# cvlab-yonsei/HVPR

Hardware: AMD Instinct MI355X
Metric: KITTI frames/sec/GPU (fwd, ~20k pts); VFE+scatter achieved HBM GB/s vs peak (higher is better)
Workload: dtype f32; 1 GPU; hvpr_car.yaml batch=1 forward-only, a1..a8 (on-GPU voxelize, pillar VFE, memory read-out + scatter, BEV backbone, head + decode, score top-k + rotated-BEV NMS); frames sharded over ranks, replicas only; global_batch=1, weights=deterministic synthetic (seed 0), BN stats randomised, cls bias -4.595

## Files before the change

### hvpr_amd/_lib.py

```python
import ctypes
import os

_HERE = os.path.dirname(os.path.abspath(__file__))
ABI_VERSION = 7
LIB_PATH = os.environ.get("HVPR_AMD_LIB", os.path.join(_HERE, "libhvpr_amd.so"))

_c = ctypes
_P = _c.c_void_p
_I = _c.c_int
_F = _c.c_float
_Z = _c.c_size_t
ALLREDUCE_FN = _c.CFUNCTYPE(_I, _P, _I, _P, _P)

SIGNATURES = {
    "hvpr_abi_version": (_I, []),
    "hvpr_status_string": (_c.c_char_p, [_I]),
    "hvpr_set_batchnorm_allreduce": (None, [_P, _P]),
    "hvpr_voxelize_workspace_bytes": (_Z, [_I, _I, _I, _I, _I]),
    "hvpr_voxelize_workspace_reset": (_I, [_P, _Z, _I, _I, _I, _I, _I, _P]),
    "hvpr_voxelize_workspace_status": (_I, [_P, _Z, _I, _I, _I, _I, _I, _P]),
    "hvpr_voxelize_f32": (_I, [_P, _I, _I, _I, _I, _P, _I, _F, _F, _F, _F, _F, _F, _I, _I, _I, _I, _I, _I,
                               _P, _P, _P, _P, _I, _P, _Z, _I, _I, _P]),
    "hvpr_pillar_vfe_fwd_f32": (_I, [_P, _P, _P, _I, _I, _P, _F, _F, _F, _F, _F, _F, _P, _P, _P, _P, _P, _P, _P, _P,
                                     _P, _P, _P, _P]),
# ... 37 lines not shown
    "hvpr_bn_relu_bwd_apply_nhwc_f32": (_I, [_P, _I, _I, _P, _c.c_longlong, _I, _P, _P, _P, _P, _I, _P, _P, _P, _P, _P, _c.c_double, _P]),
    "hvpr_memory_train_workspace_bytes": (_Z, [_I]),
    "hvpr_memory_train_fwd_f32": (_I, [_P, _c.c_longlong, _P, _I, _F, _P, _P, _P, _Z, _P]),
    "hvpr_memory_train_bwd_f32": (_I, [_P, _P, _c.c_longlong, _P, _I, _F, _P, _P, _P, _P, _P, _Z, _P]),
    "hvpr_point_pillar_topk_f32": (_I, [_P, _I, _P, _P, _I, _I, _P, _P]),
    "hvpr_scatter_add_rows_f32": (_I, [_P, _P, _c.c_longlong, _I, _I, _P, _P]),
    "hvpr_segment_sum_rows_f32": (_I, [_P, _c.c_longlong, _I, _I, _P, _P, _P, _c.c_longlong, _P, _c.c_longlong, _P]),
    "hvpr_fused_adam_truewd_f32": (_I, [_P, _P, _P, _P, _c.c_longlong, _F, _F, _F, _F, _F, _I, _P, _P]),
    "hvpr_assign_targets_workspace_bytes": (_Z, [_I, _I]),
    "hvpr_assign_targets_f32": (_I, [_P, _I, _P, _I, _I, _I, _I, _F, _F, _I, _I, _I, _c.c_longlong, _P, _P, _P, _P, _P, _Z, _P]),
    "hvpr_rpn_losses_workspace_bytes": (_Z, [_I, _c.c_longlong]),
    "hvpr_rpn_losses_f32": (_I, [_P, _P, _P, _P, _P, _P, _P, _I, _c.c_longlong, _I, _I, _F, _F, _F, _P, _F, _F, _F, _F, _P, _P, _P, _P,
                                 _P, _Z, _P]),
    "hvpr_mse_loss_workspace_bytes": (_Z, []),
    "hvpr_mse_loss_f32": (_I, [_P, _P, _c.c_longlong, _I, _F, _P, _P, _P, _Z, _P]),
    "hvpr_split_bf16_f32": (_I, [_P, _c.c_longlong, _I, _P, _P]),
    "hvpr_unsplit_bf16_f32": (_I, [_P, _c.c_longlong, _I, _P, _P]),
    "hvpr_conv2d_nhwc_bf16x3": (_I, [_P, _I, _I, _I, _I, _P, _P, _I, _I, _I, _I, _P, _P, _I, _P, _I, _I, _I, _I, _I, _P]),
    "hvpr_deconv_nhwc_bf16x3": (_I, [_P, _I, _I, _I, _I, _P, _P, _I, _I, _I, _I, _P, _I, _I, _I, _P]),
    "hvpr_point_flags_f32": (_I, [_P, _I, _I, _I, _P, _F, _P, _P, _I, _I, _P, _P]),
    "hvpr_compact_workspace_bytes": (_Z, [_I]),
    "hvpr_compact_rows_f32": (_I, [_P, _I, _I, _P, _P, _I, _P, _P, _Z, _P]),
    "hvpr_frame_offsets_f32": (_I, [_P, _I, _I, _I, _P, _P]),
    "hvpr_gather_rows_f32": (_I, [_P, _I, _I, _P, _I, _P, _P]),
    "hvpr_pillar_vfe_train_workspace_bytes": (_Z, []),
    "hvpr_pillar_vfe_train_fwd_f32": (_I, [_P, _P, _P, _I, _I, _P, _P, _P, _P, _P, _P, _F, _F, _F, _F, _F, _F, _F, _P, _P, _P, _P, _P, _P, _Z, _P]),
    "hvpr_pillar_vfe_bwd_f32": (_I, [_P, _P, _P, _I, _I, _P, _P, _P, _P, _P, _P, _F, _F, _F, _F, _F, _F, _F, _P, _P, _P, _P, _P, _P, _P, _P, _Z, _P]),
    "hvpr_conv2d_wino_wgrad_workspace_bytes": (_Z, [_I, _I, _I, _I, _I]),
    "hvpr_conv2d_wino_wgrad_nhwc_f32": (_I, [_P, _I, _I, _I, _I, _P, _I, _P, _P, _Z, _P]),
    "hvpr_conv2d_wino_packed_floats": (_Z, [_I, _I]),
    "hvpr_conv2d_wino_pack_f32": (_I, [_P, _P, _I, _I, _I, _P, _P]),
    "hvpr_conv2d_wino_nhwc_f32": (_I, [_P, _I, _I, _I, _I, _P, _P, _I, _I, _P, _P, _I, _P, _I, _I, _I, _P, _P]),
    "hvpr_conv2d_wino_stats_rows": (_I, [_I, _I, _I]),
    "hvpr_conv2d_s2_dgrad_nhwc_f32": (_I, [_P, _I, _I, _I, _I, _P, _P, _I, _I, _I, _I, _P, _I, _I, _P]),
    "hvpr_bn_train_affine_f32": (_I, [_P, _P, _P, _I, _P, _P, _F, _F, _P, _P, _P, _P, _P, _P]),
    "hvpr_bn_finalize_partials_f32": (_I, [_P, _I, _I, _c.c_longlong, _F, _P, _P, _P, _P]),
    "hvpr_conv2d_nhwc_f32": (_I, [_P, _I, _I, _I, _I, _P, _P, _I, _I, _I, _I, _I, _I, _P, _P, _I, _P, _I, _I, _I, _P]),
}

_lib = None


class HvprLibraryError(RuntimeError):
    pass


def lib():
    global _lib
    if _lib is None:
        if not os.path.exists(LIB_PATH):
            raise HvprLibraryError(
                f"{LIB_PATH} is missing: build it with `python -m hvpr_amd.build` (hipcc --offload-arch=gfx950). "
                "hvpr_amd has no CPU fallback.")
        try:
            L = ctypes.CDLL(LIB_PATH)
        except OSError as e:
            raise HvprLibraryError(f"cannot load {LIB_PATH}: {e}") from e
        for name, (res, args) in SIGNATURES.items():
            fn = getattr(L, name)
            fn.restype = res
            fn.argtypes = args
        if L.hvpr_abi_version() != ABI_VERSION:
            raise HvprLibraryError(f"{LIB_PATH} has ABI version {L.hvpr_abi_version()}, these wrappers need {ABI_VERSION}: "
                                   "rebuild it with `python -m hvpr_amd.build`")
        _lib = L
    return _lib
# ... 7 lines not shown
```

### hvpr_amd/bev_backbone.py

```python
import contextlib
import os

import torch
import torch.nn as nn

from . import kernels
from .folding import FoldCache, bn_scale_shift


class ConvLayer(nn.Module):

    def __init__(self, in_channels, out_channels, kernel_size, stride=1, padding=0, use_norm=True, activation=False):
        super().__init__()
        self.conv = nn.Conv2d(in_channels, out_channels, kernel_size=kernel_size, stride=stride, padding=padding)
        self.norm = nn.BatchNorm2d(out_channels, eps=1e-3, momentum=0.01) if use_norm else None
        self.relu = nn.ReLU() if activation else None


class SpatialAttention(nn.Module):

    def __init__(self):
        super().__init__()
        self.spatial = ConvLayer(2, 1, 3, stride=1, padding=1, use_norm=True, activation=False)

# ... 100 lines not shown
            cfg = _tile_cfg("trunk", i)
            lv = {"convs": []}
            sc, sh = bn_scale_shift(blk[2])
            wg = _wino_groups(i)
            lv["convs"].append(kernels.pack_conv_auto(blk[1].weight, sc, sh, stride=s, tile_cfg=cfg, px_groups=wg))
            for k in range(self.layer_nums[i]):
                sc, sh = bn_scale_shift(blk[5 + 3 * k])
                lv["convs"].append(kernels.pack_conv_auto(blk[4 + 3 * k].weight, sc, sh, tile_cfg=cfg, px_groups=wg))
            sc, sh = bn_scale_shift(self.sfmblocks_down[i][1])
            lv["sfm"] = kernels.pack_conv_auto(self.sfmblocks_down[i][0].weight, sc, sh, tile_cfg=_tile_cfg("sfm", i), px_groups=wg)
            planes = self.PRECISIONS[self.conv_precision]
            if planes:
                c3 = 4
                lv["convs3"] = []
                sc, sh = bn_scale_shift(blk[2])
                lv["convs3"].append(kernels.pack_conv_bf3(blk[1].weight, sc, sh, stride=s, tile_cfg=c3, planes=planes))
                for k in range(self.layer_nums[i]):
                    sc, sh = bn_scale_shift(blk[5 + 3 * k])
                    lv["convs3"].append(kernels.pack_conv_bf3(blk[4 + 3 * k].weight, sc, sh, tile_cfg=c3, planes=planes))
                sc, sh = bn_scale_shift(self.sfmblocks_down[i][1])
                lv["sfm3"] = kernels.pack_conv_bf3(self.sfmblocks_down[i][0].weight, sc, sh, tile_cfg=c3, planes=planes)
                de = self.deblocks[i]
                sc, sh = bn_scale_shift(de[1])
                lv["deconv3"] = kernels.pack_deconv_bf3(de[0].weight, sc, sh, planes=planes) \
                    if (planes == 2 and de[0].weight.shape[0] % 64 == 0) else None
            sl = self.scale_layers[i]
            sc, sh = bn_scale_shift(sl[2])
            lv["scale"] = kernels.pack_conv_auto(sl[1].weight, sc, sh, stride=s, tile_cfg=_tile_cfg("scale", i), px_groups=wg)
            de = self.deblocks[i]
            sc, sh = bn_scale_shift(de[1])
            us = int(self.upsample_strides[i])
            dcfg = _tile_cfg("deconv", i)
            lv["deconv"] = kernels.pack_deconv(de[0].weight, sc, sh, tile_cfg=dcfg)
            packed["levels"].append(lv)
        return packed

    def _forward_train(self, data_dict):
        if not data_dict["spatial_features"].is_cuda:
            raise RuntimeError("hvpr_amd: BaseBEVBackbone_Scale's training forward needs GPU tensors (the HIP path has no CPU fallback)")
        from . import conv_train as ct

        def nhwc(t):
            return t.permute(0, 2, 3, 1).contiguous()

        def cbr(seq, t, gate=None, resid=None):
            mods, k = list(seq), 0
            while k < len(mods):
                if isinstance(mods[k], nn.ZeroPad2d):
                    k += 1
                conv, bn = mods[k], mods[k + 1]
                last = k + 3 >= len(mods)
                if last and gate is not None and resid is t and conv.stride[0] == 1 and conv.kernel_size[0] == 3:
                    t = ct.sfm_step(t, conv.weight, bn, gate)
                else:
                    z, partials = ct.conv(t, conv.weight, conv.stride[0], stats=True)
                    t = ct.bn_relu(z, bn, gate=gate if last else None, resid=resid if last else None, partials=partials)
                k += 3
            return t

        def gate(y, uses):
            sp = self.attention.spatial
            g, mean, var = ct.spatial_gate_train(y, sp.conv.weight, sp.conv.bias, sp.norm.weight, sp.norm.bias, sp.norm.eps)
            ct.update_running_repeated(sp.norm, mean, var, ct.global_count(y.numel() // y.shape[-1], y.device), uses)
            return g

        x, xp = nhwc(data_dict["spatial_features"]), nhwc(data_dict["spatial_features_point"])
# ... 149 lines not shown
```

### hvpr_amd/csrc/conv_wino.hip

```cpp
#include <type_traits>

#include "common.h"

namespace {

typedef float f32x16 __attribute__((ext_vector_type(16)));
constexpr int KC = 8;
constexpr int BN = 64;
constexpr int TW = 16, PW = TW + 2;
constexpr int ROWP = 20;
constexpr int W_V4 = 16 * 2 * BN;

__device__ __forceinline__ void lds_dma16(const void *sbase_uniform, unsigned voff_bytes, unsigned lds_dst_uniform) {
    unsigned keep;
    asm volatile("s_mov_b32 %0, m0\n\ts_mov_b32 m0, %3\n\ts_nop 0\n\tglobal_load_lds_dwordx4 %1, %2\n\ts_mov_b32 m0, %0"
                 : "=&s"(keep)
                 : "v"(voff_bytes), "s"(sbase_uniform), "s"(lds_dst_uniform)
                 : "memory");
}

__device__ __forceinline__ unsigned lds_addr_of(const void *p) {
    return (unsigned)(size_t)(const __attribute__((address_space(3))) void *)p;
}

struct WinoArgs {
    const float *in;
    const float *wpk;
    const float *bias;
    float *out;
    const float *gate;
    const float *resid;
    int N, H, W, Cin;
    int cout, cout_pad;
    int out_cstride, out_coff, resid_cstride;
    int relu;
    int tiles_x, tiles_y, n_ct;
    float *stats;
};

__device__ __forceinline__ float4 f4_fma(float s, float4 a, float4 b) {
    return make_float4(fmaf(s, a.x, b.x), fmaf(s, a.y, b.y), fmaf(s, a.z, b.z), fmaf(s, a.w, b.w));
}
__device__ __forceinline__ float4 f4_add(float4 a, float4 b) { return make_float4(a.x + b.x, a.y + b.y, a.z + b.z, a.w + b.w); }
__device__ __forceinline__ float4 f4_sub(float4 a, float4 b) { return make_float4(a.x - b.x, a.y - b.y, a.z - b.z, a.w - b.w); }

template <int NG, bool STATS, int NB>
__global__ void __launch_bounds__(256 * NG) __attribute__((amdgpu_waves_per_eu(2, NB == 2 ? 2 : 3))) k_wino(WinoArgs a) {
    constexpr int NT = 256 * NG;
    constexpr int TH = 8 * NG, PH = TH + 2;
    constexpr int PPAD = (PH * ROWP + 63) / 64 * 64;
    constexpr int PATCH_V4 = 2 * PPAD;
    constexpr int BNT = 32 * NB, W_V4T = 16 * 2 * BNT;
    constexpr int NLD_P = (PATCH_V4 + NT - 1) / NT, NLD_W = W_V4T / NT;
    constexpr int PATCH_PAD = NLD_P * NT;
    static_assert(W_V4T % NT == 0 && (NB == 2 || NG == 1), "whole DMA pieces");
    extern __shared__ __attribute__((aligned(16))) float4 smem[];
    float4 *const s_w = smem;
    float4 *const s_patch = smem + 2 * W_V4T;

    const int tid = threadIdx.x, lane = tid & 63, wid = tid >> 6;
    const unsigned wave_s = __builtin_amdgcn_readfirstlane((unsigned)(threadIdx.x >> 6));
    const int grp = wid >> 2, wa = wid & 3;
    const int half = lane >> 5, l31 = lane & 31;
    const int by = l31 >> 3, bx = l31 & 7;

    int p_py[NLD_P], p_px[NLD_P], p_part[NLD_P];
    bool p_live[NLD_P];
#pragma unroll
    for (int i = 0; i < NLD_P; ++i) {
        const int v = tid + i * NT;
        const int plane = v / PPAD, slot = v % PPAD;
        const int y = slot / ROWP, rem = slot % ROWP;
        const int x = 2 * (rem % 10) + rem / 10;
        p_py[i] = y; p_px[i] = x; p_part[i] = plane * 4;
        p_live[i] = plane < 2 && y < PH && x < PW;
    }
    const int r0 = wa == 0 ? 0 : (wa == 2 ? 2 : 1), r1 = wa == 2 ? 1 : (wa == 3 ? 3 : 2);
    const float sgn = wa == 1 ? 1.f : -1.f;
    const int pbase = half * PPAD + (2 * (4 * grp + by)) * ROWP + bx;
    const int p_off0 = pbase + r0 * ROWP, p_off1 = pbase + r1 * ROWP;
    const int u_off = (wa * 4 * 2 + half) * BNT + l31;
    const unsigned lds_w0 = lds_addr_of(s_w) + wave_s * 1024u;
    const unsigned lds_patch0 = lds_addr_of(s_patch) + wave_s * 1024u;

    const int n_pt = a.tiles_x * a.tiles_y * a.N;
    const int total_walk = ((n_pt + 7) / 8) * 8 * a.n_ct;
    const int n_chunks = a.Cin / KC;
    for (int it = blockIdx.x; it < total_walk; it += gridDim.x) {
    const int xcd = it & 7, j = it >> 3;
    const int ct = j % a.n_ct;
    int pt = (j / a.n_ct) * 8 + xcd;
    if (pt >= n_pt) continue;
    const int tx = pt % a.tiles_x; pt /= a.tiles_x;
    const int ty = pt % a.tiles_y;
    const int n = pt / a.tiles_y;
    const int oy0 = ty * TH, ox0 = tx * TW;
    const int iy0 = oy0 - 1, ix0 = ox0 - 1;
    const int co0 = ct * BNT;

    unsigned poff[NLD_P];
    bool pok[NLD_P];
#pragma unroll
    for (int i = 0; i < NLD_P; ++i) {
        const int iy = iy0 + p_py[i], ix = ix0 + p_px[i];
        pok[i] = p_live[i] && iy >= 0 && iy < a.H && ix >= 0 && ix < a.W;
        poff[i] = pok[i] ? (unsigned)(((iy * a.W + ix) * a.Cin + p_part[i]) * (int)sizeof(float)) : 0u;
    }
    const char *in_n = (const char *)(a.in + (size_t)n * a.H * a.W * a.Cin);
    const char *w_ct = (const char *)(a.wpk + (size_t)(NB == 2 ? ct : ct >> 1) * n_chunks * (W_V4 * 4));
    const unsigned w_half = NB == 2 ? 0u : (unsigned)(ct & 1) * 32u * 16u;

    auto stage_piece = [&](int chunk, int buf, int i) {
        if (i < NLD_P) {
            const char *pbase_g = in_n + (size_t)chunk * (KC * sizeof(float));
            if (pok[i]) lds_dma16(pbase_g, poff[i], lds_patch0 + (unsigned)(buf * PATCH_PAD + i * NT) * 16u);
        } else {
            const int j = i - NLD_P;
            const char *wbase = w_ct + (size_t)chunk * (W_V4 * 16);
            lds_dma16(wbase, NB == 2 ? (unsigned)((tid + j * NT) * 16) : (unsigned)((((tid + j * NT) >> 5) * 64 + ((tid + j * NT) & 31)) * 16) + w_half,
                      lds_w0 + (unsigned)(buf * W_V4T + j * NT) * 16u);
        }
    };
    auto stage = [&](int chunk, int buf) {
#pragma unroll
        for (int i = 0; i < NLD_P + NLD_W; ++i) stage_piece(chunk, buf, i);
    };
    const bool border = iy0 < 0 || ix0 < 0 || iy0 + PH > a.H || ix0 + PW > a.W;
    if (border) {
#pragma unroll
        for (int b = 0; b < 2; ++b)
#pragma unroll
            for (int i = 0; i < NLD_P; ++i) s_patch[b * PATCH_PAD + tid + i * NT] = make_float4(0.f, 0.f, 0.f, 0.f);
        __syncthreads();
    }
    static_assert(PH * ROWP + BNT / 4 <= PPAD, "room for the bias row behind the patch");
    if (tid < BNT / 4) s_patch[PH * ROWP + tid] = *(const float4 *)(a.bias + co0 + tid * 4);
    f32x16 acc[4][NB];
#pragma unroll
    for (int b = 0; b < 4; ++b)
#pragma unroll
        for (int nb = 0; nb < NB; ++nb)
#pragma unroll
// ... 5 lines not shown
        __builtin_amdgcn_s_barrier();
        const float4 *sp = s_patch + BUF * PATCH_PAD;
        const float4 *sw = s_w + BUF * W_V4T;
        float4 d0[4], d1[4], u[4][NB];
#pragma unroll
        for (int jx = 0; jx < 4; ++jx) {
            d0[jx] = sp[p_off0 + (jx & 1) * 10 + (jx >> 1)];
            d1[jx] = sp[p_off1 + (jx & 1) * 10 + (jx >> 1)];
        }
#pragma unroll
        for (int b = 0; b < 2; ++b)
#pragma unroll
            for (int nb = 0; nb < NB; ++nb) u[b][nb] = sw[u_off + b * 2 * BNT + nb * 32];
        __builtin_amdgcn_sched_barrier(0);
        float4 t[4], v[4];
#pragma unroll
        for (int jx = 0; jx < 4; ++jx) t[jx] = f4_fma(sgn, d1[jx], d0[jx]);
        v[0] = f4_sub(t[0], t[2]); v[1] = f4_add(t[1], t[2]); v[2] = f4_sub(t[2], t[1]); v[3] = f4_sub(t[1], t[3]);
#pragma unroll
        for (int b = 0; b < 4; ++b) {
            if (b + 2 < 4) {
#pragma unroll
                for (int nb = 0; nb < NB; ++nb) u[b + 2][nb] = sw[u_off + (b + 2) * 2 * BNT + nb * 32];
            }
            __builtin_amdgcn_sched_barrier(0);
#pragma unroll
            for (int nb = 0; nb < NB; ++nb) {
                acc[b][nb] = __builtin_amdgcn_mfma_f32_32x32x2f32(u[b][nb].x, v[b].x, acc[b][nb], 0, 0, 0);
                acc[b][nb] = __builtin_amdgcn_mfma_f32_32x32x2f32(u[b][nb].y, v[b].y, acc[b][nb], 0, 0, 0);
                acc[b][nb] = __builtin_amdgcn_mfma_f32_32x32x2f32(u[b][nb].z, v[b].z, acc[b][nb], 0, 0, 0);
                acc[b][nb] = __builtin_amdgcn_mfma_f32_32x32x2f32(u[b][nb].w, v[b].w, acc[b][nb], 0, 0, 0);
                constexpr int DEAL = 4 * NB > 5 ? 5 : 4 * NB - 1, NPF = (NLD_P + NLD_W + DEAL - 1) / DEAL;
                static_assert(DEAL * NPF >= NLD_P + NLD_W, "every piece goes out");
                if (c + 1 < n_chunks && b * NB + nb < DEAL) {
                    __builtin_amdgcn_sched_barrier(0);
#pragma unroll
                    for (int i = (b * NB + nb) * NPF; i < (b * NB + nb + 1) * NPF && i < NLD_P + NLD_W; ++i) stage_piece(c + 1, BUF ^ 1, i);
                    __builtin_amdgcn_sched_barrier(0);
                }
            }
            __builtin_amdgcn_sched_barrier(0);
        }
    };
    stage(0, 0);
    for (int c = 0; c + 1 < n_chunks; c += 2) {
        chunk_step(c, std::integral_constant<int, 0>{});
        chunk_step(c + 1, std::integral_constant<int, 1>{});
    }
    if (n_chunks & 1) chunk_step(n_chunks - 1, std::integral_constant<int, 0>{});

    const int p = wa >> 1, q = wa & 1;
    const int oy = oy0 + 2 * (4 * grp + by) + p, ox = ox0 + 2 * bx + q;
    const bool live_px = oy < a.H && ox < a.W;
    const size_t pix = ((size_t)n * a.H + (live_px ? oy : 0)) * a.W + (live_px ? ox : 0);
    const float gate = a.gate && live_px ? a.gate[pix] : 0.f;
    const float *rrow = a.gate ? a.resid + pix * a.resid_cstride : nullptr;
    const float sg = p ? -1.f : 1.f;
    constexpr int NPASS = NG == 1 ? 1 : 2, NBP = NB / NPASS;
    float4 ykeep[2][4];
#pragma unroll
    for (int i = 0; i < 8; ++i) ykeep[i >> 2][i & 3] = make_float4(0.f, 0.f, 0.f, 0.f);
#pragma unroll
    for (int ps = 0; ps < NPASS; ++ps) {
        __syncthreads();
#pragma unroll
        for (int nl = 0; nl < NBP; ++nl) {
            const int nb = ps * NBP + nl;
#pragma unroll
            for (int g = 0; g < 4; ++g) {
                float4 m[4];
#pragma unroll
                for (int b = 0; b < 4; ++b) m[b] = make_float4(acc[b][nb][4 * g], acc[b][nb][4 * g + 1], acc[b][nb][4 * g + 2], acc[b][nb][4 * g + 3]);
                s_w[((((grp * 4 + wa) * 2 + 0) * NBP + nl) * 4 + g) * 64 + lane] = f4_add(f4_add(m[0], m[1]), m[2]);
                s_w[((((grp * 4 + wa) * 2 + 1) * NBP + nl) * 4 + g) * 64 + lane] = f4_sub(f4_sub(m[1], m[2]), m[3]);
            }
        }
        __syncthreads();
        if (live_px) {
#pragma unroll
            for (int nl = 0; nl < NBP; ++nl) {
                const int nb = ps * NBP + nl;
#pragma unroll
                for (int g = 0; g < 4; ++g) {
                    const int col = co0 + nb * 32 + 8 * g + 4 * half;
                    if (col >= a.cout) continue;
                    const float4 x0 = s_w[((((grp * 4 + p) * 2 + q) * NBP + nl) * 4 + g) * 64 + lane];
                    const float4 x1 = s_w[((((grp * 4 + p + 1) * 2 + q) * NBP + nl) * 4 + g) * 64 + lane];
                    const float4 x2 = s_w[((((grp * 4 + p + 2) * 2 + q) * NBP + nl) * 4 + g) * 64 + lane];
                    const float4 bias = s_patch[PH * ROWP + (col - co0) / 4];
                    float4 y = f4_add(f4_fma(sg, x2, f4_fma(sg, x1, x0)), bias);
                    if (a.relu) { y.x = fmaxf(y.x, 0.f); y.y = fmaxf(y.y, 0.f); y.z = fmaxf(y.z, 0.f); y.w = fmaxf(y.w, 0.f); }
                    if (a.gate) {
                        const float4 r = *(const float4 *)(rrow + col);
                        y.x = fmaf(gate, y.x, r.x); y.y = fmaf(gate, y.y, r.y); y.z = fmaf(gate, y.z, r.z); y.w = fmaf(gate, y.w, r.w);
                    }
                    *(float4 *)(a.out + pix * a.out_cstride + a.out_coff + col) = y;
                    if (STATS) ykeep[nl][g] = y;
                }
            }
        }
    }
    static_assert(!STATS || (NG == 1 && NB == 2), "the statistics pass is written for the 8 x 16 px x 64 channel tile");
    if (STATS) {
        __syncthreads();
#pragma unroll
        for (int nl = 0; nl < 2; ++nl)
#pragma unroll
            for (int g = 0; g < 4; ++g) s_w[((wid * 2 + nl) * 4 + g) * 64 + lane] = ykeep[nl][g];
        __syncthreads();
        {
            const int c = tid & 63, part = tid >> 6;
// ... 23 lines not shown

__global__ void k_wino_pack(const float *__restrict__ w, const float *__restrict__ scale, int cout, int cin, int cout_pad, int adjoint,
                            float *__restrict__ out) {
    const long long id = blockIdx.x * (long long)blockDim.x + threadIdx.x;
    if (id >= (long long)cout_pad * cin) return;
    const int o = (int)(id / cin), i = (int)(id % cin);
    double g[3][3];
#pragma unroll
    for (int u = 0; u < 3; ++u)
#pragma unroll
        for (int v = 0; v < 3; ++v) {
            double x = 0.0;
            if (o < cout) x = adjoint ? (double)w[(((size_t)i * cout + o) * 3 + (2 - u)) * 3 + (2 - v)] : (double)w[(((size_t)o * cin + i) * 3 + u) * 3 + v];
            g[u][v] = (scale && o < cout) ? x * (double)scale[o] : x;
        }
    double gg[4][3];
#pragma unroll
    for (int v = 0; v < 3; ++v) {
        gg[0][v] = g[0][v];
        gg[1][v] = 0.5 * (g[0][v] + g[1][v] + g[2][v]);
        gg[2][v] = 0.5 * (g[0][v] - g[1][v] + g[2][v]);
        gg[3][v] = g[2][v];
    }
    const int ct = o / BN, co_l = o % BN, chunk = i / KC, hf = (i % KC) / 4, e = i % 4;
    float *dst = out + ((size_t)ct * (cin / KC) + chunk) * (W_V4 * 4);
#pragma unroll
    for (int r = 0; r < 4; ++r) {
        const double U[4] = {gg[r][0], 0.5 * (gg[r][0] + gg[r][1] + gg[r][2]), 0.5 * (gg[r][0] - gg[r][1] + gg[r][2]), gg[r][2]};
#pragma unroll
        for (int b = 0; b < 4; ++b) dst[(((size_t)(r * 4 + b) * 2 + hf) * BN + co_l) * 4 + e] = (float)U[b];
    }
}

template <int NG, bool STATS, int NB>
int launch(WinoArgs a, hipStream_t s) {
    constexpr int NT = 256 * NG, TH = 8 * NG, PH = TH + 2;
    constexpr int PPAD = (PH * ROWP + 63) / 64 * 64;
    constexpr int NLD_P = (2 * PPAD + NT - 1) / NT;
    constexpr int lds = (2 * (16 * 2 * 32 * NB) + 2 * NLD_P * NT) * 16;
    a.tiles_x = (a.W + TW - 1) / TW;
    a.tiles_y = (a.H + TH - 1) / TH;
    a.n_ct = a.cout_pad / (32 * NB);
    static unsigned long long lds_set = 0ull;
    if (hvpr_ensure_dyn_lds((const void *)k_wino<NG, STATS, NB>, lds, &lds_set) != 0) return -1;
    const long long tiles = (long long)a.N * a.tiles_x * a.tiles_y * a.n_ct;
    static int resident = 0;
    if (resident == 0) {
        int per_cu = 0, dev = 0, cus = 256;
        hipDeviceProp_t prop;
        if (hipGetDevice(&dev) == hipSuccess && hipGetDeviceProperties(&prop, dev) == hipSuccess) cus = prop.multiProcessorCount;
        if (hipOccupancyMaxActiveBlocksPerMultiprocessor(&per_cu, k_wino<NG, STATS, NB>, NT, lds) != hipSuccess || per_cu < 1) per_cu = 1;
        resident = per_cu * cus;
    }
    long long blocks = tiles < resident ? (tiles + 7) / 8 * 8 : resident;
    if (blocks > resident && resident >= 8) blocks = resident / 8 * 8;
    hipLaunchKernelGGL((k_wino<NG, STATS, NB>), dim3((unsigned)blocks), dim3(NT), lds, s, a);
    return 0;
}

}

extern "C" int hvpr_conv2d_wino_stats_rows(int N, int H, int W) {
    if (N < 1 || H < 1 || W < 1) return 0;
    return N * ((H + 7) / 8) * ((W + TW - 1) / TW);
}

extern "C" size_t hvpr_conv2d_wino_packed_floats(int cin, int cout) {
    if (cin < 1 || cout < 1) return 0;
    return (size_t)((cout + BN - 1) / BN * BN) * (size_t)cin * 16;
}

extern "C" int hvpr_conv2d_wino_pack_f32(const float *weight, const float *scale, int cout, int cin, int adjoint, float *packed,
                                         hvpr_stream_t stream) {
    if (!weight || !packed || cout < 1 || cin < 1) return HVPR_ERR_INVALID_ARG;
    if (cin % KC != 0) return HVPR_ERR_UNSUPPORTED;
    const int cout_pad = (cout + BN - 1) / BN * BN;
    const long long n = (long long)cout_pad * cin;
    hipLaunchKernelGGL(k_wino_pack, dim3(hvpr_cdiv(n, 256)), dim3(256), 0, (hipStream_t)stream, weight, scale, cout, cin, cout_pad,
                       adjoint ? 1 : 0, packed);
    HVPR_CHECK_LAUNCH();
    return HVPR_OK;
}

extern "C" int hvpr_conv2d_wino_nhwc_f32(const float *in, int N, int H, int W, int Cin, const float *w_packed, const float *bias,
                                         int cout, int relu, const float *gate, const float *resid, int resid_cstride, float *out,
                                         int out_cstride, int out_coff, int px_groups, float *bn_partials, hvpr_stream_t stream) {
    if (!in || !w_packed || !bias || !out || N < 1 || H < 1 || W < 1 || Cin < 8 || cout < 1) return HVPR_ERR_INVALID_ARG;
    if ((gate == nullptr) != (resid == nullptr)) return HVPR_ERR_INVALID_ARG;
    if (Cin % KC != 0) return HVPR_ERR_UNSUPPORTED;
    if (cout % 4 != 0 || out_cstride % 4 != 0 || out_coff % 4 != 0 || (resid && resid_cstride % 4 != 0)) return HVPR_ERR_UNSUPPORTED;
    if ((long long)H * W * Cin * 4 >= (1ll << 31)) return HVPR_ERR_UNSUPPORTED;
    WinoArgs a;
    a.in = in; a.wpk = w_packed; a.bias = bias; a.out = out; a.gate = gate; a.resid = resid;
    a.N = N; a.H = H; a.W = W; a.Cin = Cin;
    a.cout = cout; a.cout_pad = (cout + BN - 1) / BN * BN;
    a.out_cstride = out_cstride; a.out_coff = out_coff; a.resid_cstride = resid_cstride;
    a.relu = relu;
    a.stats = bn_partials;
    if (bn_partials && (px_groups != 1 || relu || gate)) return HVPR_ERR_UNSUPPORTED;
    int rc;
    if (px_groups == 1) rc = bn_partials ? launch<1, true, 2>(a, (hipStream_t)stream) : launch<1, false, 2>(a, (hipStream_t)stream);
    else if (px_groups == 2) rc = launch<2, false, 2>(a, (hipStream_t)stream);
    else if (px_groups == 4) rc = launch<1, false, 1>(a, (hipStream_t)stream);
    else return HVPR_ERR_INVALID_ARG;
    if (rc != 0) return HVPR_ERR_LAUNCH;
    HVPR_CHECK_LAUNCH();
    return HVPR_OK;
}
```

### hvpr_amd/kernels.py

```python
import os

import torch

from ._lib import check, lib


def _stream():
    return torch.cuda.current_stream().cuda_stream


def _ptr(t, dtype=None, name="tensor"):
    if t is None:
        return None
    if not t.is_cuda:
        raise RuntimeError(f"hvpr_amd: {name} must live on the GPU (the HIP path has no CPU fallback)")
    if dtype is not None and t.dtype != dtype:
        raise TypeError(f"hvpr_amd: {name} must be {dtype}, got {t.dtype}")
    if not t.is_contiguous():
        raise ValueError(f"hvpr_amd: {name} must be contiguous")
    return t.data_ptr()


class VoxelizeWorkspace:

# ... 333 lines not shown

    def __init__(self, w, bias, taps, stride, cout, cout_pad, up, cin, relu, tile_cfg):
        self.w, self.bias, self.taps, self.stride = w, bias, taps, stride
        self.cout, self.cout_pad, self.up, self.cin, self.relu, self.tile_cfg = cout, cout_pad, up, cin, relu, tile_cfg


def _tile_channels(tile_cfg):
    return 128 if tile_cfg == 0 else 64


def pack_conv(weight, scale=None, shift=None, stride=1, relu=True, tile_cfg=0):
    cout, cin, kh, kw = weight.shape
    assert kh == kw and kh in (1, 3) and cin % 8 == 0
    w = weight.detach().float()
    if scale is not None:
        w = w * scale.view(-1, 1, 1, 1)
    tc = _tile_channels(tile_cfg)
    cout_pad = (cout + tc - 1) // tc * tc
    taps = kh * kw
    p = w.permute(2, 3, 1, 0).reshape(taps, cin // 8, 2, 4, cout).permute(0, 1, 2, 4, 3)
    wp = torch.zeros((taps, cin // 8, 2, cout_pad, 4), dtype=torch.float32, device=w.device)
    wp[:, :, :, :cout] = p
    b = torch.zeros((cout_pad,), dtype=torch.float32, device=w.device)
    if shift is not None:
        b[:cout] = shift.detach().float()
    return PackedConv(wp.contiguous(), b, taps, stride, cout, cout_pad, 1, cin, relu, tile_cfg)


_zero_bias = {}


class PackedConvWino:

    __slots__ = ("w", "bias", "cout", "cout_pad", "cin", "relu", "px_groups")
    taps, stride, up = 9, 1, 1

    def __init__(self, w, bias, cout, cout_pad, cin, relu, px_groups):
        self.w, self.bias, self.cout, self.cout_pad, self.cin, self.relu, self.px_groups = w, bias, cout, cout_pad, cin, relu, px_groups


def pack_conv_wino(weight, scale=None, shift=None, relu=True, px_groups=1, adjoint=False):
    w = weight.detach()
    if w.dtype != torch.float32 or not w.is_contiguous():
        w = w.float().contiguous()
    cout, cin = (w.shape[1], w.shape[0]) if adjoint else (w.shape[0], w.shape[1])
    assert w.shape[2:] == (3, 3) and cin % 8 == 0 and cout % 4 == 0
    cout_pad = (cout + 63) // 64 * 64
    wp = torch.empty((lib().hvpr_conv2d_wino_packed_floats(cin, cout),), dtype=torch.float32, device=w.device)
    sc = None if scale is None else scale.detach().float().contiguous()
    check(lib().hvpr_conv2d_wino_pack_f32(_ptr(w, torch.float32, "conv weight"), _ptr(sc, torch.float32, "scale"), cout, cin,
                                          1 if adjoint else 0, wp.data_ptr(), _stream()), "hvpr_conv2d_wino_pack_f32")
    if shift is None:
        key = (cout_pad, w.device)
        if key not in _zero_bias:
            _zero_bias[key] = torch.zeros((cout_pad,), dtype=torch.float32, device=w.device)
        b = _zero_bias[key]
    else:
        b = torch.zeros((cout_pad,), dtype=torch.float32, device=w.device)
        b[:cout] = shift.detach().float()
    return PackedConvWino(wp, b, cout, cout_pad, cin, relu, px_groups)


def conv2d_wino_nhwc(x, pc, out=None, out_coff=0, gate=None, resid=None, bn_partials=None):
    N, H, W, cin = x.shape
    assert cin == pc.cin
    if out is None:
        out = torch.empty((N, H, W, pc.cout), dtype=torch.float32, device=x.device)
    assert out.shape[:3] == (N, H, W) and out.is_contiguous()
    check(lib().hvpr_conv2d_wino_nhwc_f32(_ptr(x, torch.float32, "conv input"), N, H, W, cin, pc.w.data_ptr(), pc.bias.data_ptr(),
                                          pc.cout, 1 if pc.relu else 0, _ptr(gate, torch.float32, "gate"),
                                          _ptr(resid, torch.float32, "resid"), 0 if resid is None else resid.shape[-1],
                                          out.data_ptr(), out.shape[-1], int(out_coff), pc.px_groups,
                                          _ptr(bn_partials, torch.float32, "bn_partials"), _stream()), "hvpr_conv2d_wino_nhwc_f32")
    return out


def pack_deconv(weight, scale, shift, relu=True, tile_cfg=0):
    cin, cout, s, s2 = weight.shape
    assert s == s2 and cin % 8 == 0
    w = weight.detach().float() * scale.view(1, -1, 1, 1)
    cols = s * s * cout
    tc = _tile_channels(tile_cfg)
    cout_pad = (cols + tc - 1) // tc * tc
    g = w.permute(0, 2, 3, 1).reshape(cin, cols)
    p = g.reshape(cin // 8, 2, 4, cols).permute(0, 1, 3, 2).unsqueeze(0)
    wp = torch.zeros((1, cin // 8, 2, cout_pad, 4), dtype=torch.float32, device=w.device)
    wp[:, :, :, :cols] = p
    b = torch.zeros((cout_pad,), dtype=torch.float32, device=w.device)
    b[:cols] = shift.detach().float().repeat(s * s)
    return PackedConv(wp.contiguous(), b, 1, 1, cout, cout_pad, s, cin, relu, tile_cfg)


def conv_algo():
    algo = os.environ.get("HVPR_CONV_ALGO", "winograd")
    if algo not in ("winograd", "direct"):
        raise ValueError(f"HVPR_CONV_ALGO must be 'winograd' or 'direct', got {algo!r}")
    return algo


def pack_conv_auto(weight, scale=None, shift=None, stride=1, relu=True, tile_cfg=1, px_groups=1):
    if weight.shape[2] == 3 and stride == 1 and weight.shape[0] % 4 == 0 and weight.shape[1] % 8 == 0 and conv_algo() == "winograd":
# ... 125 lines not shown
```

### include/hvpr_amd.h

```cpp
#ifndef HVPR_AMD_H
#define HVPR_AMD_H

#include <stddef.h>
#include <stdint.h>

#ifdef __cplusplus
extern "C" {
#endif

typedef void *hvpr_stream_t;

enum hvpr_status {
    HVPR_OK = 0,
    HVPR_ERR_INVALID_ARG = -1,
    HVPR_ERR_UNSUPPORTED = -2,
    HVPR_ERR_WORKSPACE = -3,
    HVPR_ERR_LAUNCH = -4,
    HVPR_ERR_TIMEOUT = -5
};

int hvpr_abi_version(void);
const char *hvpr_status_string(int status);

typedef int (*hvpr_allreduce_fn)(double *buf, int n, hvpr_stream_t stream, void *ctx);
// ... 154 lines not shown
                                   float *dbeta, void *workspace, size_t workspace_bytes, hvpr_stream_t stream);
int hvpr_bn_relu_bwd_apply_nhwc_f32(const float *dy, int dy_cstride, int dy_coff, const float *z, long long P, int C, const float *scale,
                                    const float *shift, const float *mean, const float *invstd, int relu, const float *gate, float *dgate,
                                    float *dz, const float *dgamma_total, const float *dbeta_total, double inv_count, hvpr_stream_t stream);

size_t hvpr_assign_targets_workspace_bytes(int batch, int n_gt);
int hvpr_assign_targets_f32(const float *anchors, int n_anchors, const float *gt_boxes, int batch, int n_gt, int class_index,
                            int n_classes, float matched_thr, float unmatched_thr, int per_loc, int loc_stride, int loc_offset,
                            long long anchors_total, int32_t *labels, float *reg_targets, float *reg_weights, int32_t *pos_count,
                            void *workspace, size_t workspace_bytes, hvpr_stream_t stream);

size_t hvpr_rpn_losses_workspace_bytes(int batch, long long n_anchors);
int hvpr_rpn_losses_f32(const float *cls_preds, const float *box_preds, const float *dir_preds, const int32_t *labels,
                        const float *reg_targets, const float *anchor_rot, const int32_t *pos_count, int batch, long long n_anchors,
                        int num_class, int num_dir_bins, float alpha, float gamma, float beta, const float *code_weights,
                        float cls_weight, float loc_weight, float dir_weight, float dir_offset, float *losses, float *grad_cls,
                        float *grad_box, float *grad_dir, void *workspace, size_t workspace_bytes, hvpr_stream_t stream);
size_t hvpr_mse_loss_workspace_bytes(void);
int hvpr_mse_loss_f32(const float *x, const float *target, long long rows, int cols, float weight, float *loss, float *grad_x,
                      void *workspace, size_t workspace_bytes, hvpr_stream_t stream);

int hvpr_fused_adam_truewd_f32(float *params, const float *grads, float *exp_avg, float *exp_avg_sq, long long n, float lr,
                               float beta1, float beta2, float eps, float weight_decay, int step,
                               const float *grad_scale_device, hvpr_stream_t stream);


size_t hvpr_conv2d_wino_packed_floats(int cin, int cout);
int hvpr_conv2d_wino_pack_f32(const float *weight, const float *scale, int cout, int cin, int adjoint, float *packed,
                              hvpr_stream_t stream);
int hvpr_conv2d_wino_nhwc_f32(const float *in, int N, int H, int W, int Cin, const float *w_packed, const float *bias, int cout,
                              int relu, const float *gate, const float *resid, int resid_cstride, float *out, int out_cstride,
                              int out_coff, int px_groups, float *bn_partials, hvpr_stream_t stream);
int hvpr_conv2d_wino_stats_rows(int N, int H, int W);

int hvpr_split_bf16_f32(const float *src, long long n_floats, int n_planes, void *dst, hvpr_stream_t stream);
int hvpr_unsplit_bf16_f32(const void *src, long long n_floats, int n_planes, float *dst, hvpr_stream_t stream);
int hvpr_conv2d_nhwc_bf16x3(const void *in_split, int N, int H, int W, int Cin, const void *w_split, const float *bias,
                            int stride, int cout, int cout_pad, int relu, const float *gate, const void *resid_split,
                            int resid_cstride, void *out, int out_split, int out_cstride, int out_coff, int tile_cfg,
                            int n_planes, hvpr_stream_t stream);
int hvpr_deconv_nhwc_bf16x3(const void *in_split, int N, int H, int W, int Cin, const void *w_split, const float *bias, int cout,
                            int cout_pad, int up, int relu, float *out, int out_cstride, int out_coff, int n_planes,
                            hvpr_stream_t stream);

int hvpr_point_flags_f32(const float *points, int n, int stride, int mode, const float *range_xy, float near_thresh,
                         const float *fov_lidar_to_rect, const float *fov_rect_to_img, int img_h, int img_w, uint8_t *flags,
                         hvpr_stream_t stream);
size_t hvpr_compact_workspace_bytes(int n);
int hvpr_compact_rows_f32(const float *src, int n, int row_floats, const uint8_t *flags, float *dst, int capacity,
                          int32_t *count, void *workspace, size_t workspace_bytes, hvpr_stream_t stream);
int hvpr_gather_rows_f32(const float *src, int n_src, int row_floats, const int32_t *idx, int m, float *dst,
                         hvpr_stream_t stream);
int hvpr_frame_offsets_f32(const float *points, int n_points, int point_stride, int batch, int32_t *frame_offsets,
                           hvpr_stream_t stream);

#ifdef __cplusplus
}
#endif
#endif
```

Baseline: 453.7 frames/s.

## Add split-K Winograd conv path for low-occupancy BEV backbone levels

Adds a split-K variant of the Winograd conv kernel. Each output tile's input-channel reduction is divided across several workgroups, which write partial sums to a global slab, and the last arriving workgroup (found by an atomic ticket counter) reduces them and applies bias, relu and the gate epilogue. A cost model picks the split factor per layer from tile count versus resident slots, so that deep, spatially small backbone levels fill more CUs. The trade is extra slab traffic, a counter-zeroing launch, and a per-call workspace allocation.

```diff
diff --git a/hvpr_amd/_lib.py b/hvpr_amd/_lib.py
--- a/hvpr_amd/_lib.py
+++ b/hvpr_amd/_lib.py
@@ -93,6 +93,9 @@
     "hvpr_conv2d_wino_pack_f32": (_I, [_P, _P, _I, _I, _I, _P, _P]),
     "hvpr_conv2d_wino_nhwc_f32": (_I, [_P, _I, _I, _I, _I, _P, _P, _I, _I, _P, _P, _I, _P, _I, _I, _I, _P, _P]),
     "hvpr_conv2d_wino_stats_rows": (_I, [_I, _I, _I]),
+    "hvpr_conv2d_wino_ksplit": (_I, [_I, _I, _I, _I]),
+    "hvpr_conv2d_wino_splitk_workspace_bytes": (_Z, [_I, _I, _I, _I, _I, _I]),
+    "hvpr_conv2d_wino_splitk_nhwc_f32": (_I, [_P, _I, _I, _I, _I, _P, _P, _I, _I, _P, _P, _I, _P, _I, _I, _I, _P, _I, _P, _Z, _P]),
     "hvpr_conv2d_s2_dgrad_nhwc_f32": (_I, [_P, _I, _I, _I, _I, _P, _P, _I, _I, _I, _I, _P, _I, _I, _P]),
     "hvpr_bn_train_affine_f32": (_I, [_P, _P, _P, _I, _P, _P, _F, _F, _P, _P, _P, _P, _P, _P]),
     "hvpr_bn_finalize_partials_f32": (_I, [_P, _I, _I, _c.c_longlong, _F, _P, _P, _P, _P]),
diff --git a/hvpr_amd/bev_backbone.py b/hvpr_amd/bev_backbone.py
--- a/hvpr_amd/bev_backbone.py
+++ b/hvpr_amd/bev_backbone.py
@@ -156,6 +156,9 @@
             us = int(self.upsample_strides[i])
             dcfg = _tile_cfg("deconv", i)
             lv["deconv"] = kernels.pack_deconv(de[0].weight, sc, sh, tile_cfg=dcfg)
+            for pc in lv["convs"] + [lv["sfm"], lv["scale"]]:
+                if isinstance(pc, kernels.PackedConvWino):
+                    pc.ksplit = kernels.lib().hvpr_conv2d_wino_ksplit(h, w, pc.cin, pc.cout)
             packed["levels"].append(lv)
         return packed
 
diff --git a/hvpr_amd/csrc/conv_wino.hip b/hvpr_amd/csrc/conv_wino.hip
--- a/hvpr_amd/csrc/conv_wino.hip
+++ b/hvpr_amd/csrc/conv_wino.hip
@@ -36,7 +36,14 @@
     int relu;
     int tiles_x, tiles_y, n_ct;
     float *stats;
+    int ksplit;
+    float4 *slab;
+    unsigned *cnt;
 };
+
+constexpr unsigned WAIT_VM0 = 0x0F70;
+constexpr int SC1 = 16;
+typedef unsigned u32x4 __attribute__((ext_vector_type(4)));
 
 __device__ __forceinline__ float4 f4_fma(float s, float4 a, float4 b) {
     return make_float4(fmaf(s, a.x, b.x), fmaf(s, a.y, b.y), fmaf(s, a.z, b.z), fmaf(s, a.w, b.w));
@@ -44,7 +51,7 @@
 __device__ __forceinline__ float4 f4_add(float4 a, float4 b) { return make_float4(a.x + b.x, a.y + b.y, a.z + b.z, a.w + b.w); }
 __device__ __forceinline__ float4 f4_sub(float4 a, float4 b) { return make_float4(a.x - b.x, a.y - b.y, a.z - b.z, a.w - b.w); }
 
-template <int NG, bool STATS, int NB>
+template <int NG, bool STATS, int NB, bool SPLIT>
 __global__ void __launch_bounds__(256 * NG) __attribute__((amdgpu_waves_per_eu(2, NB == 2 ? 2 : 3))) k_wino(WinoArgs a) {
     constexpr int NT = 256 * NG;
     constexpr int TH = 8 * NG, PH = TH + 2;
@@ -54,6 +61,7 @@
     constexpr int NLD_P = (PATCH_V4 + NT - 1) / NT, NLD_W = W_V4T / NT;
     constexpr int PATCH_PAD = NLD_P * NT;
     static_assert(W_V4T % NT == 0 && (NB == 2 || NG == 1), "whole DMA pieces");
+    static_assert(!SPLIT || (NG == 1 && NB == 2 && !STATS), "split-K is written for the 8 x 16 px x 64 channel tile, no statistics");
     extern __shared__ __attribute__((aligned(16))) float4 smem[];
     float4 *const s_w = smem;
     float4 *const s_patch = smem + 2 * W_V4T;
@@ -84,13 +92,24 @@
     const unsigned lds_patch0 = lds_addr_of(s_patch) + wave_s * 1024u;
 
     const int n_pt = a.tiles_x * a.tiles_y * a.N;
-    const int total_walk = ((n_pt + 7) / 8) * 8 * a.n_ct;
-    const int n_chunks = a.Cin / KC;
+    const int S = SPLIT ? a.ksplit : 1;
+    const int n_grp = a.n_ct * S;
+    const bool grp_walk = SPLIT && n_grp % 8 == 0;
+    const int total_walk = grp_walk ? n_pt * n_grp : ((n_pt + 7) / 8) * 8 * n_grp;
+    const int n_chunks = a.Cin / KC, n_kc = n_chunks / S;
     for (int it = blockIdx.x; it < total_walk; it += gridDim.x) {
     const int xcd = it & 7, j = it >> 3;
-    const int ct = j % a.n_ct;
-    int pt = (j / a.n_ct) * 8 + xcd;
-    if (pt >= n_pt) continue;
+    int g, pt;
+    if (grp_walk) {
+        g = (j % (n_grp >> 3)) * 8 + xcd;
+        pt = j / (n_grp >> 3);
+    } else {
+        g = j % n_grp;
+        pt = (j / n_grp) * 8 + xcd;
+        if (pt >= n_pt) continue;
+    }
+    const int ct = g / S, ks = g % S;
+    const int tile = pt * a.n_ct + ct;
     const int tx = pt % a.tiles_x; pt /= a.tiles_x;
     const int ty = pt % a.tiles_y;
     const int n = pt / a.tiles_y;
@@ -106,8 +125,8 @@
         pok[i] = p_live[i] && iy >= 0 && iy < a.H && ix >= 0 && ix < a.W;
         poff[i] = pok[i] ? (unsigned)(((iy * a.W + ix) * a.Cin + p_part[i]) * (int)sizeof(float)) : 0u;
     }
-    const char *in_n = (const char *)(a.in + (size_t)n * a.H * a.W * a.Cin);
-    const char *w_ct = (const char *)(a.wpk + (size_t)(NB == 2 ? ct : ct >> 1) * n_chunks * (W_V4 * 4));
+    const char *in_n = (const char *)(a.in + (size_t)n * a.H * a.W * a.Cin + ks * n_kc * KC);
+    const char *w_ct = (const char *)(a.wpk + ((size_t)(NB == 2 ? ct : ct >> 1) * n_chunks + ks * n_kc) * (W_V4 * 4));
     const unsigned w_half = NB == 2 ? 0u : (unsigned)(ct & 1) * 32u * 16u;
 
     auto stage_piece = [&](int chunk, int buf, int i) {
@@ -179,7 +198,7 @@
                 acc[b][nb] = __builtin_amdgcn_mfma_f32_32x32x2f32(u[b][nb].w, v[b].w, acc[b][nb], 0, 0, 0);
                 constexpr int DEAL = 4 * NB > 5 ? 5 : 4 * NB - 1, NPF = (NLD_P + NLD_W + DEAL - 1) / DEAL;
                 static_assert(DEAL * NPF >= NLD_P + NLD_W, "every piece goes out");
-                if (c + 1 < n_chunks && b * NB + nb < DEAL) {
+                if (c + 1 < n_kc && b * NB + nb < DEAL) {
                     __builtin_amdgcn_sched_barrier(0);
 #pragma unroll
                     for (int i = (b * NB + nb) * NPF; i < (b * NB + nb + 1) * NPF && i < NLD_P + NLD_W; ++i) stage_piece(c + 1, BUF ^ 1, i);
@@ -190,11 +209,11 @@
         }
     };
     stage(0, 0);
-    for (int c = 0; c + 1 < n_chunks; c += 2) {
+    for (int c = 0; c + 1 < n_kc; c += 2) {
         chunk_step(c, std::integral_constant<int, 0>{});
         chunk_step(c + 1, std::integral_constant<int, 1>{});
     }
-    if (n_chunks & 1) chunk_step(n_chunks - 1, std::integral_constant<int, 0>{});
+    if (n_kc & 1) chunk_step(n_kc - 1, std::integral_constant<int, 0>{});
 
     const int p = wa >> 1, q = wa & 1;
     const int oy = oy0 + 2 * (4 * grp + by) + p, ox = ox0 + 2 * bx + q;
@@ -223,7 +242,63 @@
             }
         }
         __syncthreads();
-        if (live_px) {
+        if constexpr (SPLIT) {
+            const __amdgpu_buffer_rsrc_t rs = __builtin_amdgcn_make_buffer_rsrc(a.slab + (size_t)tile * S * (8 * NT), (short)0,
+                                                                                S * (int)(8 * NT * sizeof(float4)), 0x00020000);
+#pragma unroll
+            for (int nl = 0; nl < 2; ++nl)
+#pragma unroll
+                for (int g = 0; g < 4; ++g) {
+                    const float4 x0 = s_w[((((grp * 4 + p) * 2 + q) * 2 + nl) * 4 + g) * 64 + lane];
+                    const float4 x1 = s_w[((((grp * 4 + p + 1) * 2 + q) * 2 + nl) * 4 + g) * 64 + lane];
+                    const float4 x2 = s_w[((((grp * 4 + p + 2) * 2 + q) * 2 + nl) * 4 + g) * 64 + lane];
+                    const float4 r = f4_fma(sg, x2, f4_fma(sg, x1, x0));
+                    const u32x4 v = {__float_as_uint(r.x), __float_as_uint(r.y), __float_as_uint(r.z), __float_as_uint(r.w)};
+                    __builtin_amdgcn_raw_buffer_store_b128(v, rs, tid * 16, (ks * 8 + nl * 4 + g) * NT * 16, SC1);
+                }
+            __builtin_amdgcn_s_waitcnt(WAIT_VM0);
+            __syncthreads();
+            int *const s_last = (int *)s_w;
+            if (tid == 0) {
+                const unsigned ticket = __hip_atomic_fetch_add(a.cnt + tile, 1u, __ATOMIC_RELAXED, __HIP_MEMORY_SCOPE_AGENT);
+                const int last = ticket == (unsigned)(S - 1);
+                if (last) __hip_atomic_store(a.cnt + tile, 0u, __ATOMIC_RELAXED, __HIP_MEMORY_SCOPE_AGENT);
+                *s_last = last;
+            }
+            __syncthreads();
+            if (__builtin_amdgcn_readfirstlane(*s_last)) {
+                auto ld = [&](int k, int i) {
+                    const u32x4 v = __builtin_amdgcn_raw_buffer_load_b128(rs, tid * 16, (k * 8 + i) * NT * 16, SC1);
+                    return make_float4(__uint_as_float(v.x), __uint_as_float(v.y), __uint_as_float(v.z), __uint_as_float(v.w));
+                };
+                float4 y[8];
+#pragma unroll
+                for (int i = 0; i < 8; ++i) y[i] = ld(0, i);
+                for (int k = 1; k < S; ++k) {
+                    float4 v[8];
+#pragma unroll
+                    for (int i = 0; i < 8; ++i) v[i] = ld(k, i);
+#pragma unroll
+                    for (int i = 0; i < 8; ++i) y[i] = f4_add(y[i], v[i]);
+                }
+                if (live_px) {
+#pragma unroll
+                    for (int nl = 0; nl < 2; ++nl)
+#pragma unroll
+                        for (int g = 0; g < 4; ++g) {
+                            const int col = co0 + nl * 32 + 8 * g + 4 * half;
+                            if (col >= a.cout) continue;
+                            float4 r = f4_add(y[nl * 4 + g], s_patch[PH * ROWP + (col - co0) / 4]);
+                            if (a.relu) { r.x = fmaxf(r.x, 0.f); r.y = fmaxf(r.y, 0.f); r.z = fmaxf(r.z, 0.f); r.w = fmaxf(r.w, 0.f); }
+                            if (a.gate) {
+                                const float4 rs = *(const float4 *)(rrow + col);
+                                r.x = fmaf(gate, r.x, rs.x); r.y = fmaf(gate, r.y, rs.y); r.z = fmaf(gate, r.z, rs.z); r.w = fmaf(gate, r.w, rs.w);
+                            }
+                            *(float4 *)(a.out + pix * a.out_cstride + a.out_coff + col) = r;
+                        }
+                }
+            }
+        } else if (live_px) {
 #pragma unroll
             for (int nl = 0; nl < NBP; ++nl) {
                 const int nb = ps * NBP + nl;
@@ -313,30 +388,58 @@
     }
 }
 
-template <int NG, bool STATS, int NB>
-int launch(WinoArgs a, hipStream_t s) {
+__global__ void k_zero_counters(unsigned *cnt, int n) {
+    const int i = blockIdx.x * blockDim.x + threadIdx.x;
+    if (i < n) __hip_atomic_store(cnt + i, 0u, __ATOMIC_RELAXED, __HIP_MEMORY_SCOPE_AGENT);
+}
+
+template <int NG, int NB>
+constexpr int lds_bytes() {
     constexpr int NT = 256 * NG, TH = 8 * NG, PH = TH + 2;
     constexpr int PPAD = (PH * ROWP + 63) / 64 * 64;
     constexpr int NLD_P = (2 * PPAD + NT - 1) / NT;
-    constexpr int lds = (2 * (16 * 2 * 32 * NB) + 2 * NLD_P * NT) * 16;
-    a.tiles_x = (a.W + TW - 1) / TW;
-    a.tiles_y = (a.H + TH - 1) / TH;
-    a.n_ct = a.cout_pad / (32 * NB);
+    return (2 * (16 * 2 * 32 * NB) + 2 * NLD_P * NT) * 16;
+}
+
+template <int NG, bool STATS, int NB, bool SPLIT>
+int resident_slots() {
+    constexpr int lds = lds_bytes<NG, NB>();
     static unsigned long long lds_set = 0ull;
-    if (hvpr_ensure_dyn_lds((const void *)k_wino<NG, STATS, NB>, lds, &lds_set) != 0) return -1;
-    const long long tiles = (long long)a.N * a.tiles_x * a.tiles_y * a.n_ct;
+    if (hvpr_ensure_dyn_lds((const void *)k_wino<NG, STATS, NB, SPLIT>, lds, &lds_set) != 0) return 0;
     static int resident = 0;
     if (resident == 0) {
         int per_cu = 0, dev = 0, cus = 256;
         hipDeviceProp_t prop;
         if (hipGetDevice(&dev) == hipSuccess && hipGetDeviceProperties(&prop, dev) == hipSuccess) cus = prop.multiProcessorCount;
-        if (hipOccupancyMaxActiveBlocksPerMultiprocessor(&per_cu, k_wino<NG, STATS, NB>, NT, lds) != hipSuccess || per_cu < 1) per_cu = 1;
+        if (hipOccupancyMaxActiveBlocksPerMultiprocessor(&per_cu, k_wino<NG, STATS, NB, SPLIT>, 256 * NG, lds) != hipSuccess || per_cu < 1) per_cu = 1;
         resident = per_cu * cus;
     }
-    long long blocks = tiles < resident ? (tiles + 7) / 8 * 8 : resident;
+    return resident;
+}
+
+template <int NG, bool STATS, int NB, bool SPLIT = false>
+int launch(WinoArgs a, hipStream_t s) {
+    constexpr int NT = 256 * NG, TH = 8 * NG, lds = lds_bytes<NG, NB>();
+    a.tiles_x = (a.W + TW - 1) / TW;
+    a.tiles_y = (a.H + TH - 1) / TH;
+    a.n_ct = a.cout_pad / (32 * NB);
+    const int resident = resident_slots<NG, STATS, NB, SPLIT>();
+    if (resident == 0) return -1;
+    const long long tiles = (long long)a.N * a.tiles_x * a.tiles_y * a.n_ct;
+    const long long units = SPLIT ? tiles * a.ksplit : tiles;
+    if (SPLIT) hipLaunchKernelGGL(k_zero_counters, dim3(hvpr_cdiv(tiles, 256)), dim3(256), 0, s, a.cnt, (int)tiles);
+    long long blocks = units < resident ? (units + 7) / 8 * 8 : resident;
     if (blocks > resident && resident >= 8) blocks = resident / 8 * 8;
-    hipLaunchKernelGGL((k_wino<NG, STATS, NB>), dim3((unsigned)blocks), dim3(NT), lds, s, a);
+    hipLaunchKernelGGL((k_wino<NG, STATS, NB, SPLIT>), dim3((unsigned)blocks), dim3(NT), lds, s, a);
     return 0;
+}
+
+constexpr int KSPLIT_MAX = 8;
+constexpr size_t SLAB_BYTES = 8 * 256 * sizeof(float4);
+
+size_t splitk_counter_offset(int N, int H, int W, int cout, int ksplit) {
+    const size_t tiles = (size_t)N * ((H + 7) / 8) * ((W + TW - 1) / TW) * ((cout + BN - 1) / BN);
+    return tiles * ksplit * SLAB_BYTES;
 }
 
 }
@@ -363,9 +466,44 @@
     return HVPR_OK;
 }
 
+extern "C" size_t hvpr_conv2d_wino_splitk_workspace_bytes(int N, int H, int W, int Cin, int cout, int ksplit) {
+    if (N < 1 || H < 1 || W < 1 || Cin < KC || cout < 1 || ksplit <= 1) return 0;
+    const size_t tiles = (size_t)N * ((H + 7) / 8) * ((W + TW - 1) / TW) * ((cout + BN - 1) / BN);
+    return splitk_counter_offset(N, H, W, cout, ksplit) + tiles * sizeof(unsigned);
+}
+
+extern "C" int hvpr_conv2d_wino_ksplit(int H, int W, int Cin, int cout) {
+    if (H < 1 || W < 1 || Cin < KC || Cin % KC != 0 || cout < 1) return 1;
+    constexpr double C0 = 16.0;
+    const int R = resident_slots<1, false, 2, true>();
+    if (R <= 0) return 1;
+    const long long T = (long long)((H + 7) / 8) * ((W + TW - 1) / TW) * ((cout + BN - 1) / BN);
+    const int C = Cin / KC;
+    int best = 1;
+    double best_t = 1e300;
+    for (int S = 1; S <= KSPLIT_MAX && C % S == 0; S *= 2) {
+        const double t = (double)((T * S + R - 1) / R) * ((double)C / S + C0);
+        if (t < best_t) best = S, best_t = t;
+    }
+    return best;
+}
+
+extern "C" int hvpr_conv2d_wino_splitk_nhwc_f32(const float *in, int N, int H, int W, int Cin, const float *w_packed, const float *bias,
+                                                int cout, int relu, const float *gate, const float *resid, int resid_cstride, float *out,
+                                                int out_cstride, int out_coff, int px_groups, float *bn_partials, int ksplit,
+                                                void *workspace, size_t workspace_bytes, hvpr_stream_t stream);
+
 extern "C" int hvpr_conv2d_wino_nhwc_f32(const float *in, int N, int H, int W, int Cin, const float *w_packed, const float *bias,
                                          int cout, int relu, const float *gate, const float *resid, int resid_cstride, float *out,
                                          int out_cstride, int out_coff, int px_groups, float *bn_partials, hvpr_stream_t stream) {
+    return hvpr_conv2d_wino_splitk_nhwc_f32(in, N, H, W, Cin, w_packed, bias, cout, relu, gate, resid, resid_cstride, out, out_cstride,
+                                            out_coff, px_groups, bn_partials, 1, nullptr, 0, stream);
+}
+
+extern "C" int hvpr_conv2d_wino_splitk_nhwc_f32(const float *in, int N, int H, int W, int Cin, const float *w_packed, const float *bias,
+                                                int cout, int relu, const float *gate, const float *resid, int resid_cstride, float *out,
+                                                int out_cstride, int out_coff, int px_groups, float *bn_partials, int ksplit,
+                                                void *workspace, size_t workspace_bytes, hvpr_stream_t stream) {
     if (!in || !w_packed || !bias || !out || N < 1 || H < 1 || W < 1 || Cin < 8 || cout < 1) return HVPR_ERR_INVALID_ARG;
     if ((gate == nullptr) != (resid == nullptr)) return HVPR_ERR_INVALID_ARG;
     if (Cin % KC != 0) return HVPR_ERR_UNSUPPORTED;
@@ -378,9 +516,19 @@
     a.out_cstride = out_cstride; a.out_coff = out_coff; a.resid_cstride = resid_cstride;
     a.relu = relu;
     a.stats = bn_partials;
+    a.ksplit = 1; a.slab = nullptr; a.cnt = nullptr;
     if (bn_partials && (px_groups != 1 || relu || gate)) return HVPR_ERR_UNSUPPORTED;
+    if (ksplit < 1) return HVPR_ERR_INVALID_ARG;
     int rc;
-    if (px_groups == 1) rc = bn_partials ? launch<1, true, 2>(a, (hipStream_t)stream) : launch<1, false, 2>(a, (hipStream_t)stream);
+    if (ksplit > 1) {
+        if (bn_partials || px_groups != 1 || ksplit > KSPLIT_MAX || (Cin / KC) % ksplit != 0) return HVPR_ERR_UNSUPPORTED;
+        if (!workspace || workspace_bytes < hvpr_conv2d_wino_splitk_workspace_bytes(N, H, W, Cin, cout, ksplit)) return HVPR_ERR_INVALID_ARG;
+        if ((size_t)workspace % 16 != 0) return HVPR_ERR_INVALID_ARG;
+        a.ksplit = ksplit;
+        a.slab = (float4 *)workspace;
+        a.cnt = (unsigned *)((char *)workspace + splitk_counter_offset(N, H, W, cout, ksplit));
+        rc = launch<1, false, 2, true>(a, (hipStream_t)stream);
+    } else if (px_groups == 1) rc = bn_partials ? launch<1, true, 2>(a, (hipStream_t)stream) : launch<1, false, 2>(a, (hipStream_t)stream);
     else if (px_groups == 2) rc = launch<2, false, 2>(a, (hipStream_t)stream);
     else if (px_groups == 4) rc = launch<1, false, 1>(a, (hipStream_t)stream);
     else return HVPR_ERR_INVALID_ARG;
diff --git a/hvpr_amd/kernels.py b/hvpr_amd/kernels.py
--- a/hvpr_amd/kernels.py
+++ b/hvpr_amd/kernels.py
@@ -389,11 +389,12 @@
 
 class PackedConvWino:
 
-    __slots__ = ("w", "bias", "cout", "cout_pad", "cin", "relu", "px_groups")
+    __slots__ = ("w", "bias", "cout", "cout_pad", "cin", "relu", "px_groups", "ksplit")
     taps, stride, up = 9, 1, 1
 
-    def __init__(self, w, bias, cout, cout_pad, cin, relu, px_groups):
+    def __init__(self, w, bias, cout, cout_pad, cin, relu, px_groups, ksplit=1):
         self.w, self.bias, self.cout, self.cout_pad, self.cin, self.relu, self.px_groups = w, bias, cout, cout_pad, cin, relu, px_groups
+        self.ksplit = ksplit
 
 
 def pack_conv_wino(weight, scale=None, shift=None, relu=True, px_groups=1, adjoint=False):
@@ -424,6 +425,15 @@
     if out is None:
         out = torch.empty((N, H, W, pc.cout), dtype=torch.float32, device=x.device)
     assert out.shape[:3] == (N, H, W) and out.is_contiguous()
+    if pc.ksplit > 1:
+        nbytes = lib().hvpr_conv2d_wino_splitk_workspace_bytes(N, H, W, cin, pc.cout, pc.ksplit)
+        ws = torch.empty((nbytes,), dtype=torch.uint8, device=x.device)
+        check(lib().hvpr_conv2d_wino_splitk_nhwc_f32(
+            _ptr(x, torch.float32, "conv input"), N, H, W, cin, pc.w.data_ptr(), pc.bias.data_ptr(), pc.cout, 1 if pc.relu else 0,
+            _ptr(gate, torch.float32, "gate"), _ptr(resid, torch.float32, "resid"), 0 if resid is None else resid.shape[-1],
+            out.data_ptr(), out.shape[-1], int(out_coff), pc.px_groups, _ptr(bn_partials, torch.float32, "bn_partials"), pc.ksplit,
+            ws.data_ptr(), nbytes, _stream()), "hvpr_conv2d_wino_splitk_nhwc_f32")
+        return out
     check(lib().hvpr_conv2d_wino_nhwc_f32(_ptr(x, torch.float32, "conv input"), N, H, W, cin, pc.w.data_ptr(), pc.bias.data_ptr(),
                                           pc.cout, 1 if pc.relu else 0, _ptr(gate, torch.float32, "gate"),
                                           _ptr(resid, torch.float32, "resid"), 0 if resid is None else resid.shape[-1],
diff --git a/include/hvpr_amd.h b/include/hvpr_amd.h
--- a/include/hvpr_amd.h
+++ b/include/hvpr_amd.h
@@ -210,6 +210,12 @@
                               int relu, const float *gate, const float *resid, int resid_cstride, float *out, int out_cstride,
                               int out_coff, int px_groups, float *bn_partials, hvpr_stream_t stream);
 int hvpr_conv2d_wino_stats_rows(int N, int H, int W);
+int hvpr_conv2d_wino_ksplit(int H, int W, int Cin, int cout);
+size_t hvpr_conv2d_wino_splitk_workspace_bytes(int N, int H, int W, int Cin, int cout, int ksplit);
+int hvpr_conv2d_wino_splitk_nhwc_f32(const float *in, int N, int H, int W, int Cin, const float *w_packed, const float *bias,
+                                     int cout, int relu, const float *gate, const float *resid, int resid_cstride, float *out,
+                                     int out_cstride, int out_coff, int px_groups, float *bn_partials, int ksplit, void *workspace,
+                                     size_t workspace_bytes, hvpr_stream_t stream);
 
 int hvpr_split_bf16_f32(const float *src, long long n_floats, int n_planes, void *dst, hvpr_stream_t stream);
 int hvpr_unsplit_bf16_f32(const void *src, long long n_floats, int n_planes, float *dst, hvpr_stream_t stream);
```

Result: no change. 453.8 frames/s (median of 6 runs) (+0.0%).
